# atenpas/gpd

Hardware: AMD Instinct MI355X
Metric: 15-ch grasp candidates scored/sec (imagegen+LeNet) at 1/2/4/8 MI355X (higher is better)
Workload: dtype f64 geometry / u8 images / LeNet f32-equivalent by exact operand splitting: conv1 int8 digit planes of 32-bit fixed-point weights (i32 accumulate, exact), conv2 + ip1 three bf16 pieces per operand (six exact products per term, f32 accumulate), ip2 f32

## Files before the change

### gpd_amd/api.py

```python
import ctypes as C
import os
import subprocess

import numpy as np

_HERE = os.path.dirname(os.path.abspath(__file__))
LIB_PATH = os.environ.get("GPD_HIP_LIB") or os.path.join(_HERE, "libgpd_hip.so")
_LIB = None

HAND_DTYPE = np.dtype([
    ("sample", "<f8", (3,)), ("frame", "<f8", (9,)), ("position", "<f8", (3,)),
    ("top", "<f8"), ("bottom", "<f8"), ("center", "<f8"), ("grasp_width", "<f8"),
    ("score", "<f4"), ("finger_placement_index", "<i4"), ("set_index", "<i4"), ("slot", "<i4"),
    ("valid", "u1"), ("half_antipodal", "u1"), ("full_antipodal", "u1"), ("pad_", "u1", (5,)),
], align=False)


class Params(C.Structure):
    _fields_ = [
        ("finger_width", C.c_double), ("hand_outer_diameter", C.c_double), ("hand_depth", C.c_double),
        ("hand_height", C.c_double), ("init_bite", C.c_double), ("volume_width", C.c_double),
        ("volume_depth", C.c_double), ("volume_height", C.c_double), ("nn_radius_frames", C.c_double),
        ("friction_coeff", C.c_double), ("min_aperture", C.c_double), ("max_aperture", C.c_double),
        ("workspace_grasps", C.c_double * 6), ("image_size", C.c_int32), ("image_num_channels", C.c_int32),
# ... 126 lines not shown
    rc = lib().gpd_hip_sis_select(_ptr(cen) if len(cen) else None, len(cen), _ptr(g) if len(g) else None, len(g),
                                  _ptr(u) if len(u) else None, len(u), _ptr(lst) if lst is not None and len(lst) else None,
                                  0 if lst is None else len(lst), _ptr(xyz) if len(xyz) else None, len(xyz), _ptr(ws),
                                  int(sampling_method), int(num_gauss), int(num_rand), _ptr(samples), _ptr(acc), _ptr(used), C.byref(short))
    if rc != 0:
        raise GpdHipError("libgpd_hip error %d: %s" % (rc, lib().gpd_hip_last_error().decode()))
    return dict(samples=samples[:n].copy(), accepted=acc, consumed=used, shortfall=int(short.value))


class ImageModel(C.Structure):
    _fields_ = [("window_class", C.c_int32), ("set_sd", C.c_int32), ("set_sr", C.c_int32), ("num_shadow", C.c_int32),
                ("stride_a", C.c_uint32), ("stride_c", C.c_uint32), ("true_div", C.c_int32), ("reserved_", C.c_int32),
                ("thr", (C.c_double * 61) * 3)]


def image_model(params):
    m = ImageModel()
    rc = lib().gpd_hip_image_model(C.byref(params), C.byref(m))
    if rc != 0:
        raise GpdHipError("libgpd_hip error %d: %s" % (rc, lib().gpd_hip_last_error().decode()))
    out = {k: int(getattr(m, k)) for k in ("window_class", "set_sd", "set_sr", "num_shadow", "stride_a", "stride_c", "true_div")}
    out["thr"] = np.array(m.thr, np.float64).reshape(3, 61)
    return out


TORCH_KEYS = ("conv1.weight", "conv1.bias", "conv2.weight", "conv2.bias", "fc1.weight", "fc1.bias", "fc2.weight", "fc2.bias")


def torch_state_arrays(state):
    plain = {}
    for k, v in state.items():
        k = str(k)
        plain[k[len("module."):] if k.startswith("module.") else k] = v
    out = {}
    for k in TORCH_KEYS:
        if k not in plain:
            raise KeyError("state dict has no %r (keys: %s)" % (k, sorted(plain)))
        v = plain[k]
        if hasattr(v, "detach"):
            v = v.detach().cpu().numpy()
        out[k] = np.ascontiguousarray(v, np.float32)
    return out


def lenet_from_torch(state, channels, input_scale=1.0 / 256):
    t = torch_state_arrays(state)
# ... 86 lines not shown
    if rc != 0:
        raise GpdHipError("libgpd_hip error %d: %s" % (rc, L.gpd_hip_last_error().decode()))
    return shape, outs


def bind_host_thread(device):
    n = C.c_int(0)
    node = lib().gpd_hip_bind_host_thread(int(device), C.byref(n))
    return int(node), int(n.value)


EXPORTS = ["gpd_hip_default_params", "gpd_hip_create", "gpd_hip_destroy", "gpd_hip_last_error",
           "gpd_hip_set_lenet_weights", "gpd_hip_score", "gpd_hip_upload_cloud", "gpd_hip_search",
           "gpd_hip_images", "gpd_hip_detect", "gpd_hip_last_stage_ms", "gpd_hip_replay", "gpd_hip_replay_times", "gpd_hip_last_images_stats", "gpd_hip_estimate_normals",
           "gpd_hip_search_samples", "gpd_hip_detect_samples", "gpd_hip_reevaluate", "gpd_hip_replay_kernel_ms", "gpd_hip_last_centre_chains",
           "gpd_hip_detect_select", "gpd_hip_detect_batch", "gpd_hip_detect_batch_multi", "gpd_hip_conv1_stats", "gpd_hip_last_fallbacks", "gpd_hip_preprocess_cloud", "gpd_hip_find_clusters", "gpd_hip_reserve", "gpd_hip_bind_host_thread",
           "gpd_hip_set_lenet_mode", "gpd_hip_lenet_debug", "gpd_hip_lenet_fast_tables", "gpd_hip_detect_sharded",
           "gpd_hip_sample_above_plane", "gpd_hip_last_image_routes", "gpd_hip_refine_normals", "gpd_hip_sample_positions",
           "gpd_hip_set_lenet_conv_relu", "gpd_hip_lenet_from_torch",
           "gpd_hip_lenet_shape_check", "gpd_hip_lenet_net_from_torch", "gpd_hip_set_lenet_net", "gpd_hip_lenet_net_debug",
           "gpd_hip_lenet_net_info", "gpd_hip_set_lenet_net_mode", "gpd_hip_bf16_split3",
           "gpd_hip_upload_ground_truth", "gpd_hip_label_view", "gpd_hip_balance_view", "gpd_hip_sizeof_label_view_job",
           "gpd_hip_shuffle_orders", "gpd_hip_sis_proposals", "gpd_hip_sis_select", "gpd_hip_detect_sis", "gpd_hip_sizeof_sis_job",
           "gpd_hip_image_model", "gpd_hip_given_check", "gpd_hip_images_given", "gpd_hip_score_given",
           "gpd_hip_train_default_params", "gpd_hip_train_create", "gpd_hip_train_destroy", "gpd_hip_train_init_state",
           "gpd_hip_train_set_state", "gpd_hip_train_get_state", "gpd_hip_train_set_data", "gpd_hip_train_steps",
           "gpd_hip_train_gradients", "gpd_hip_train_apply", "gpd_hip_train_eval", "gpd_hip_train_step_timed",
           "gpd_hip_train_kernel_name", "gpd_hip_sizeof_train_recipe", "gpd_hip_train_default_recipe", "gpd_hip_train_create_recipe",
           "gpd_hip_train_init_xavier", "gpd_hip_train_learning_rate", "gpd_hip_train_get_solver_state",
           "gpd_hip_train_set_solver_state", "gpd_hip_train_kernel_name_of",
           "gpd_hip_train_reserve", "gpd_hip_train_count", "gpd_hip_train_append_data", "gpd_hip_train_get_data",
           "gpd_hip_train_reorder", "gpd_hip_train_append_view",
           "gpd_hip_train_group_mean", "gpd_hip_train_group_slices", "gpd_hip_train_group_schedule", "gpd_hip_train_group_create",
           "gpd_hip_train_group_destroy", "gpd_hip_train_group_broadcast", "gpd_hip_train_group_steps", "gpd_hip_train_group_verify",
           "gpd_hip_train_group_last_bytes",
           "gpd_hip_train_create_net", "gpd_hip_train_shape", "gpd_hip_train_net_set_state", "gpd_hip_train_net_get_state",
           "gpd_hip_train_net_gradients", "gpd_hip_train_net_apply", "gpd_hip_train_net_get_solver_state",
           "gpd_hip_train_net_set_solver_state", "gpd_hip_train_net_sizes", "gpd_hip_train_net_init_state",
           "gpd_hip_train_net_init_xavier"]


def build(prof=True):
    subprocess.check_call(["make", "-s", "-j4", "-C", os.path.join(_HERE, "csrc")])
    if prof:
        subprocess.check_call(["make", "-s", "-j4", "-C", os.path.join(_HERE, "csrc"), "prof"])


# ... 43 lines not shown
        L.gpd_hip_reserve.argtypes = [C.c_void_p, C.c_int, C.c_int, C.c_int, C.c_int, C.c_int]
        L.gpd_hip_bind_host_thread.argtypes = [C.c_int, C.POINTER(C.c_int)]
        L.gpd_hip_set_lenet_mode.argtypes = [C.c_void_p, C.c_int]
        L.gpd_hip_set_lenet_conv_relu.argtypes = [C.c_void_p, C.c_int]
        L.gpd_hip_lenet_from_torch.argtypes = [C.c_int, C.c_double] + [C.c_void_p] * 6
        L.gpd_hip_lenet_debug.argtypes = [C.c_void_p, C.c_int, C.c_int, C.c_void_p]
        L.gpd_hip_lenet_shape_check.argtypes = [C.POINTER(LenetShape)]
        L.gpd_hip_lenet_net_from_torch.argtypes = [C.POINTER(LenetShape), C.c_double, C.c_void_p, C.c_void_p]
        L.gpd_hip_set_lenet_net.argtypes = [C.c_void_p, C.POINTER(LenetShape), C.c_void_p]
        L.gpd_hip_lenet_net_debug.argtypes = [C.c_void_p, C.c_int, C.c_int, C.c_void_p]
        L.gpd_hip_lenet_net_info.argtypes = [C.c_void_p, C.c_void_p]
        L.gpd_hip_set_lenet_net_mode.argtypes = [C.c_void_p, C.c_int]
        L.gpd_hip_bf16_split3.argtypes = [C.c_void_p, C.c_longlong, C.c_void_p, C.c_void_p, C.c_void_p]
        L.gpd_hip_replay_times.argtypes = [C.c_void_p, C.c_void_p, C.POINTER(C.c_int), C.c_void_p]
        L.gpd_hip_upload_ground_truth.argtypes = [C.c_void_p, C.c_void_p, C.c_void_p, C.c_int]
        L.gpd_hip_label_view.argtypes = [C.c_void_p, C.POINTER(LabelViewJob)]
        L.gpd_hip_balance_view.argtypes = [C.c_void_p, C.c_int, C.c_int, C.c_void_p, C.POINTER(C.c_int), C.POINTER(C.c_int)]
        L.gpd_hip_shuffle_orders.argtypes = [C.c_uint32, C.c_void_p, C.c_int, C.c_void_p]
        L.gpd_hip_sis_proposals.argtypes = [C.c_uint32, C.c_int, C.c_int, C.c_longlong, C.c_int, C.c_double, C.c_void_p]
        L.gpd_hip_sis_select.argtypes = [C.c_void_p, C.c_int, C.c_void_p, C.c_int, C.c_void_p, C.c_int, C.c_void_p, C.c_int, C.c_void_p, C.c_int,
                                         C.c_void_p, C.c_int, C.c_int, C.c_int, C.c_void_p, C.c_void_p, C.c_void_p, C.POINTER(C.c_int)]
        L.gpd_hip_detect_sis.argtypes = [C.c_void_p, C.POINTER(SisJob)]
        L.gpd_hip_image_model.argtypes = [C.POINTER(Params), C.POINTER(ImageModel)]
        L.gpd_hip_given_check.argtypes = [C.POINTER(Params), C.c_void_p, C.c_int, C.POINTER(C.c_int), C.POINTER(C.c_int)]
        L.gpd_hip_images_given.argtypes = [C.c_void_p, C.c_void_p, C.c_int, C.c_uint64, C.c_void_p, C.c_void_p, C.POINTER(C.c_int),
                                           C.POINTER(C.c_uint64)]
        L.gpd_hip_score_given.argtypes = [C.c_void_p, C.c_void_p, C.c_int, C.c_uint64, C.c_void_p, C.c_void_p, C.POINTER(C.c_int),
                                          C.POINTER(C.c_uint64)]
        L.gpd_hip_train_default_params.argtypes = [C.POINTER(TrainParams)]
        L.gpd_hip_train_default_params.restype = None
        L.gpd_hip_train_create.argtypes = [C.c_void_p, C.POINTER(TrainParams), C.POINTER(C.c_void_p)]
        L.gpd_hip_train_destroy.argtypes = [C.c_void_p]
        L.gpd_hip_train_destroy.restype = None
        L.gpd_hip_train_init_state.argtypes = [C.c_int, C.c_uint32, C.POINTER(C.c_void_p)]
        L.gpd_hip_train_set_state.argtypes = [C.c_void_p, C.POINTER(C.c_void_p)]
        L.gpd_hip_train_get_state.argtypes = [C.c_void_p, C.POINTER(C.c_void_p)]
        L.gpd_hip_train_set_data.argtypes = [C.c_void_p, C.c_int, C.c_void_p, C.c_void_p, C.c_int]
        L.gpd_hip_train_steps.argtypes = [C.c_void_p, C.c_void_p, C.c_int, C.c_int, C.c_void_p]
        L.gpd_hip_train_gradients.argtypes = [C.c_void_p, C.c_void_p, C.c_int, C.POINTER(C.c_void_p), C.POINTER(C.c_float)]
        L.gpd_hip_train_apply.argtypes = [C.c_void_p, C.POINTER(C.c_void_p)]
        L.gpd_hip_train_eval.argtypes = [C.c_void_p, C.c_int, C.c_void_p, C.c_int, C.c_void_p, C.POINTER(C.c_int)]
        L.gpd_hip_train_step_timed.argtypes = [C.c_void_p, C.c_void_p, C.c_int, C.c_void_p, C.c_int, C.POINTER(C.c_int)]
        L.gpd_hip_train_kernel_name.argtypes = [C.c_int]
        L.gpd_hip_train_kernel_name.restype = C.c_char_p
        L.gpd_hip_train_default_recipe.argtypes = [C.POINTER(TrainRecipe), C.c_int]
        L.gpd_hip_train_create_recipe.argtypes = [C.c_void_p, C.POINTER(TrainParams), C.POINTER(TrainRecipe), C.POINTER(C.c_void_p)]
# ... 874 lines not shown
```

### gpd_amd/csrc/image_device.h

```cpp
#pragma once
#include <cfloat>
#include <type_traits>

#include "gpd_internal.h"
#include "image_model.h"
#include "wave_ops.h"

namespace gpd {

static_assert(kImgCells == kImg, "image_model.h and gpd_internal.h disagree about the image size");
constexpr int IMG_THREADS = 512;
constexpr int IMG_WAVES = IMG_THREADS / 64;

struct Box {
  double F[9];
  double sample[3];
  double off[3];
  double lo[3], hi[3];
};

struct PointArrays {
  double t[3][PT_CAP];
  float4 an[PT_CAP];
};
// ... 73 lines not shown
  const int h = pr == 2 ? cx : cy;
  return h + v * kImg;
}
__device__ inline int depth_axis(int pr) { return pr == 0 ? 2 : (pr == 1 ? 0 : 1); }

__device__ inline double div_len(double x, int axis) {
  const ImgConsts &K = c_img;
  if (K.true_div) return x / K.len[axis];
  const double y = K.inv_len[axis];
  const double q = x * y;
  const double r = __builtin_fma(-K.len[axis], q, x);
  return __builtin_fma(r, y, q);
}
template <int NTAB>
__device__ inline double recip_count(const double *tab, float fc) {
  const int k = (int)fc;
  return k < NTAB ? tab[k] : 1.0 / (double)fc;
}

__device__ inline uint32_t lcg_step(uint32_t &s) {
  s = 214013u * s + 2531011u;
  return (uint32_t)(((int32_t)s >> 16) & 0x7FFF);
}
__device__ inline uint32_t lcg_jump(uint32_t s, unsigned long long n) {
  const image::LcgMap m = image::lcg_affine(n);
  return m.a * s + m.c;
}

template <class SM>
__device__ inline int block_excl_scan(SM &S, int v, int *total) {
  const int lane = threadIdx.x & 63, wave = threadIdx.x >> 6;
  const int incl = wave_incl_scan_i32(v);
  if (lane == 63) S.red_i[wave] = incl;
  __syncthreads();
  int base = 0, tot = 0;
#pragma unroll
  for (int w = 0; w < IMG_WAVES; w++) {
    const int x = S.red_i[w];
    if (w < wave) base += x;
    tot += x;
  }
  *total = tot;
  return base + incl - v;
}

template <class SM>
__device__ int scan_cells(SM &S) {
  const int tid = threadIdx.x;
  constexpr int PER = 8;
  static_assert(kPix % PER == 0 && kPix / PER <= IMG_THREADS, "scan_cells: cells per thread");
// ... 404 lines not shown
```

### gpd_amd/csrc/image_model.h

```cpp
#pragma once
#include <cfloat>
#include <cmath>
#include <cstddef>
#include <cstdint>
#include <cstdio>
#include <cstring>
#include <mutex>

#include "../../include/gpd_hip.h"

namespace gpd {

constexpr int kImgCells = 60;

constexpr int SET_THREADS = 1024;
constexpr int PT_CAP = 1024;
constexpr int PT_CAP_BIG = 32768;
constexpr int SH_CAP = 6144;
constexpr int SH_CAP_BIG = 12288;
template <bool WIDE>
struct Vox {
  static constexpr int VD = WIDE ? 64 : 46;
  static constexpr int SD = WIDE ? 128 : 86;
  static constexpr int SR = WIDE ? 64 : 43;
  static constexpr int LB = 18;
  static constexpr int SETWORDS = (SD * SD * SD + 31) / 32;
};
constexpr int LGRID = 256;
constexpr size_t PTS_SCRATCH_BYTES = (size_t)PT_CAP_BIG * (3 * sizeof(double) + 4 * sizeof(float) + sizeof(uint32_t));
constexpr int HUGE_CAP = 65535;
constexpr int HUGE_WIN = 256;
constexpr size_t HUGE_SCRATCH_BYTES = (size_t)HUGE_WIN * HUGE_WIN * sizeof(int32_t) + (size_t)(HUGE_CAP + 1) * (2 * sizeof(uint32_t) + sizeof(uint16_t)) + 64;

struct ImgConsts {
  double vol_depth, vol_width, vol_height, half_od, dbl_h;
  int C, nproj, per;
  double shadow_length, voxel, voxel_mult, rand_inv;
  int num_shadow;
  uint32_t stride_a, stride_c;
  double len[3];
  double inv_cell[3];
  double thr[3][kImgCells + 1];
  double inv_len[3];
  int true_div;
  int set_sd, set_sr;
};

namespace image {

struct LcgMap {
  uint32_t a, c;
};
constexpr LcgMap lcg_affine(unsigned long long n) {
  uint32_t a = 214013u, c = 2531011u, A = 1u, Cc = 0u;
  while (n) {
    if (n & 1ull) {
      A = a * A;
      Cc = a * Cc + c;
    }
    c = (a + 1u) * c;
    a = a * a;
    n >>= 1;
  }
  return LcgMap{A, Cc};
}

struct Window {
  bool wide = false;
  bool huge = false;
  int set_sd = 0, set_sr = 0;
  int cls() const { return huge ? 2 : (wide ? 1 : 0); }
};
inline int window_class(const gpd_params &p, Window &w, char *msg, size_t msg_len) {
  const double vox = 0.003;
  const double diag = std::sqrt(p.volume_depth * p.volume_depth + p.volume_width * p.volume_width + 4.0 * p.volume_height * p.volume_height);
  const double rx = std::fmax(p.hand_depth - p.init_bite, p.volume_depth);
  const double ry = 0.5 * (p.hand_outer_diameter - p.finger_width) + 0.5 * p.volume_width;
  const double reach = std::sqrt(rx * rx + ry * ry + p.volume_height * p.volume_height);
  const double need_win = std::ceil(diag / vox) + 3.0, need_reach = std::ceil(reach / vox) + 1.0;
  w.wide = need_win > (double)Vox<false>::VD || need_reach > (double)(Vox<false>::SR - 1);
  w.huge = need_win > (double)Vox<true>::VD || need_reach > (double)(Vox<true>::SR - 1);
  if (w.huge) {
    if (need_reach + 2.0 > 640.0) {
      snprintf(msg, msg_len, "images: an image volume with %.2f m of reach is beyond the shadow region this library allocates", reach);
      return GPD_ERR_CAPACITY;
    }
    w.set_sr = (int)need_reach + 2;
    w.set_sd = 2 * w.set_sr;
// ... 70 lines not shown
  k.num_shadow = (int)std::floor(k.shadow_length / k.voxel);
  k.len[0] = k.vol_depth;
  k.len[1] = k.vol_width;
  k.len[2] = k.dbl_h;
  k.true_div = 0;
  k.set_sd = w.set_sd;
  k.set_sr = w.set_sr;
  {
    static Axis cache[3];
    static std::mutex cache_mutex;
    std::lock_guard<std::mutex> lock(cache_mutex);
    for (int a = 0; a < 3; a++) {
      Axis &ac = cache[a];
      if (ac.len != k.len[a]) axis_model(k.len[a], ac);
      k.inv_cell[a] = (double)kImgCells / k.len[a];
      std::memcpy(k.thr[a], ac.thr, sizeof(ac.thr));
      k.inv_len[a] = ac.inv_len;
      if (ac.true_div) k.true_div = 1;
    }
  }
  const LcgMap stride = lcg_affine((unsigned long long)SET_THREADS * (unsigned)k.num_shadow);
  k.stride_a = stride.a;
  k.stride_c = stride.c;
}

}
}
```

### gpd_amd/csrc/image_state.hip

```cpp
#include <cstdio>
#include <cstring>

#include <vector>

#include "gpd_internal.h"
#include "buffers.h"
#include "image_model.h"

namespace gpd {

void images_free(ImageState &im) {
  device_release(im.d_images, im.d_images_hwc, im.d_status, im.d_set_bits, im.d_overflow, im.d_overflow2, im.d_pts_overflow, im.d_pts_scratch, im.d_huge_scratch);
  if (im.ev_fork) (void)hipEventDestroy(im.ev_fork);
  if (im.ev_join) (void)hipEventDestroy(im.ev_join);
  if (im.aux) (void)hipStreamDestroy(im.aux);
  im = ImageState();
}

int images_reserve(const gpd_params &p, ImageState &im, int n, int shadow_sets) {
  const int C = p.image_num_channels;
  if (!im.d_status) {
    HIP_RET(device_alloc(im.d_status, 4));
    HIP_RET(hipMemset(im.d_status, 0, 4 * sizeof(int32_t)));
    HIP_RET(device_alloc(im.d_pts_scratch, (size_t)LGRID * PTS_SCRATCH_BYTES));
// ... 126 lines not shown
    return GPD_ERR_INVALID;
  }
  image::Window w;
  char msg[160];
  const int rc = image::window_class(*params, w, msg, sizeof(msg));
  if (rc) {
    set_error("%s", msg);
    return rc;
  }
  ImgConsts k;
  image::fill_consts(*params, w, k);
  static_assert(sizeof(out->thr) == sizeof(k.thr), "gpd_image_model");
  out->window_class = w.cls();
  out->set_sd = k.set_sd;
  out->set_sr = k.set_sr;
  out->num_shadow = k.num_shadow;
  out->stride_a = k.stride_a;
  out->stride_c = k.stride_c;
  out->true_div = k.true_div;
  out->reserved_ = 0;
  std::memcpy(out->thr, k.thr, sizeof(k.thr));
  return GPD_OK;
}
```

### gpd_amd/csrc/images.hip

```cpp
#include <cfloat>
#include <cmath>
#include <cstddef>
#include <cstdio>
#include <cstdlib>
#include <cstring>

#include <mutex>

#include "const_block.h"
#include "gpd_internal.h"
#include "image_model.h"

namespace gpd {

__constant__ ImgConsts c_img;

struct ImgParams {
  const float *nn;
  int cap;
  const double *centers;
  const gpd_hand *hands;
  const int32_t *cand_hand;
  const int32_t *meta;
  const uint32_t *set_bits;
// ... 922 lines not shown
      __syncthreads();
      const int q = it / np;
      grasp_image_body<true>(P, S, P.cand_list[q], it - q * np);
    }
  } else {
    const int cand = xcd_candidate(P.num_cand);
    if (cand < 0) return;
    grasp_image_body<false>(P, S, cand);
  }
}

struct SetParams {
  const float *nn;
  int cap;
  const double *centers;
  const double *frames;
  const int32_t *set_meta;
  uint32_t *set_bits;
  const gpd_hand *hands;
  const int32_t *hand_cand;
  int slots;
  unsigned long long lcg_base;
  double view_point[3 * kMaxCams];
};

template <int MODE>
__global__ __launch_bounds__(SET_THREADS, MODE == 0 ? 8 : 1) void shadow_set_kernel(SetParams P) {
  constexpr bool WIDE = MODE != 0;
  const ImgConsts &K = c_img;
  const int SD = MODE == 2 ? K.set_sd : Vox<MODE == 1>::SD, SR = MODE == 2 ? K.set_sr : Vox<MODE == 1>::SR;
  const int SETWORDS = MODE == 2 ? (int)(((long long)SD * SD * SD + 31) / 32) : Vox<MODE == 1>::SETWORDS;
  __shared__ uint32_t lds_bits[WIDE ? 1 : Vox<false>::SETWORDS];
  __shared__ int s_bb[6];
  const int set = blockIdx.x;
  const int tid = threadIdx.x;
  const int slot_s = P.set_meta[8 * set + 0];
  const int N = P.set_meta[8 * set + 1];
  const unsigned long long off =
      P.lcg_base + (((unsigned long long)(uint32_t)P.set_meta[8 * set + 3] << 32) | (uint32_t)P.set_meta[8 * set + 2]);
  const int cam = P.set_meta[8 * set + 4];
  const float *nn = P.nn + (size_t)slot_s * 6 * P.cap;
  uint32_t *out = P.set_bits + (size_t)set * SETWORDS;
  uint32_t *bits = WIDE ? out : lds_bits;
  if (!WIDE) {
    if (tid == 0) {
      s_bb[0] = s_bb[2] = s_bb[4] = SD;
      s_bb[1] = s_bb[3] = s_bb[5] = -1;
    }
    for (int w = tid; w < SETWORDS; w += SET_THREADS) lds_bits[w] = 0u;
    __syncthreads();
  }
  const double *smp = P.frames + 12 * (size_t)slot_s;
  const int org[3] = {(int)floor(smp[0] * K.voxel_mult) - SR, (int)floor(smp[1] * K.voxel_mult) - SR,
                      (int)floor(smp[2] * K.voxel_mult) - SR};
  if (!WIDE) {
    if (tid < P.slots && P.hand_cand[(size_t)slot_s * P.slots + tid] >= 0) {
      const gpd_hand &H = P.hands[(size_t)slot_s * P.slots + tid];
      const double lo[3] = {H.bottom, H.center - K.half_od, -1.0 * K.vol_height};
      const double hi[3] = {H.bottom + K.vol_depth, H.center + K.half_od, K.vol_height};
      double wmin[3] = {DBL_MAX, DBL_MAX, DBL_MAX}, wmax[3] = {-DBL_MAX, -DBL_MAX, -DBL_MAX};
      for (int k = 0; k < 8; k++) {
        const double bx = (k & 1) ? hi[0] : lo[0], by = (k & 2) ? hi[1] : lo[1], bz = (k & 4) ? hi[2] : lo[2];
        for (int a = 0; a < 3; a++) {
          const double w = H.sample[a] + H.frame[3 * a] * bx + H.frame[3 * a + 1] * by + H.frame[3 * a + 2] * bz;
          wmin[a] = fmin(wmin[a], w);
          wmax[a] = fmax(wmax[a], w);
        }
      }
      for (int a = 0; a < 3; a++) {
        atomicMin(&s_bb[2 * a], (int)floor(wmin[a] * K.voxel_mult) - 1 - org[a]);
        atomicMax(&s_bb[2 * a + 1], (int)floor(wmax[a] * K.voxel_mult) + 1 - org[a]);
      }
    }
    __syncthreads();
  }
  const double *cen = P.centers + 3 * (size_t)slot_s;
  double vec[3];
  for (int r = 0; r < 3; r++) vec[r] = cen[r] - P.view_point[3 * cam + r];
  const double nrm = sqrt(vec[0] * vec[0] + vec[1] * vec[1] + vec[2] * vec[2]);
  for (int r = 0; r < 3; r++) vec[r] = K.shadow_length * vec[r] / nrm;
  uint32_t state = lcg_jump(0u, off + (unsigned long long)tid * (unsigned)K.num_shadow);
  int ox = org[0], oy = org[1], oz = org[2];
  asm volatile("" : "+v"(ox), "+v"(oy), "+v"(oz));
  auto draw_ray = [&](const double p0, const double p1, const double p2, uint32_t st) {
    for (int k = 0; k < K.num_shadow; k++) {
      const double t = (double)(int)lcg_step(st) * K.rand_inv;
      const int vx = (int)((p0 + t * vec[0]) * K.voxel_mult) - ox;
      const int vy = (int)((p1 + t * vec[1]) * K.voxel_mult) - oy;
      const int vz = (int)((p2 + t * vec[2]) * K.voxel_mult) - oz;
      if ((unsigned)vx < (unsigned)SD && (unsigned)vy < (unsigned)SD && (unsigned)vz < (unsigned)SD) {
        unsigned bit;
        asm("v_mad_u32_u24 %0, %1, %2, %3" : "=v"(bit) : "v"(vx), "s"(SD), "v"(vy));
        asm("v_mad_u32_u24 %0, %1, %2, %3" : "=v"(bit) : "v"(bit), "s"(SD), "v"(vz));
        atomicOr(&bits[bit >> 5], 1u << (bit & 31));
      }
    }
  };
  if constexpr (MODE == 0) {
    double wlo[3], whi[3], dinv[3];
    bool par[3];
#pragma unroll
    for (int a = 0; a < 3; a++) {
      const int b0 = max(s_bb[2 * a], 0), b1 = min(s_bb[2 * a + 1], SD - 1);
      wlo[a] = (double)(b0 + org[a] - 2);
// ... 21 lines not shown
          const double ta = (wlo[a] - q) * dinv[a], tb = (whi[a] - q) * dinv[a];
          t0 = fmax(t0, fmin(ta, tb));
          t1 = fmin(t1, fmax(ta, tb));
        }
      }
      keep = keep && t0 <= t1;
      const unsigned long long ballot = __ballot(keep);
      const int k = __popcll(ballot);
      if (k) {
        const int below = __popcll(ballot & ((1ull << lane) - 1ull));
        const int dest = ((keep ? pend + below : pend + k + (lane - below)) & 63) << 2;
        auto move = [dest](const double x) {
          return __hiloint2double(__builtin_amdgcn_ds_permute(dest, __double2hiint(x)),
                                  __builtin_amdgcn_ds_permute(dest, __double2loint(x)));
        };
        const double a0 = move(p0), a1 = move(p1), a2 = move(p2);
        const uint32_t as = (uint32_t)__builtin_amdgcn_ds_permute(dest, (int)state);
        const bool arrived = ((lane - pend) & 63) < k;
        if (pend + k < 64) {
          if (arrived) g0 = a0, g1 = a1, g2 = a2, gs = as;
          pend += k;
        } else {
          if (lane >= pend) g0 = a0, g1 = a1, g2 = a2, gs = as;
          draw_ray(g0, g1, g2, gs);
          pend += k - 64;
          if (lane < pend) g0 = a0, g1 = a1, g2 = a2, gs = as;
        }
      }
      state = K.stride_a * state + K.stride_c;
    }
    if (lane < pend) draw_ray(g0, g1, g2, gs);
  } else {
    for (int i = tid; i < N; i += SET_THREADS) {
      draw_ray((double)nn[0 * P.cap + i], (double)nn[1 * P.cap + i], (double)nn[2 * P.cap + i], state);
      state = K.stride_a * state + K.stride_c;
    }
  }
  if (!WIDE) {
    __syncthreads();
    const int x0 = max(s_bb[0], 0), x1 = min(s_bb[1], SD - 1), y0 = max(s_bb[2], 0), y1 = min(s_bb[3], SD - 1);
    if (x1 >= x0 && y1 >= y0) {
      const int wpr = (((y1 - y0 + 1) * SD + 31) >> 5) + 1;
      for (int idx = tid; idx < (x1 - x0 + 1) * wpr; idx += SET_THREADS) {
        const int x = x0 + idx / wpr, k = idx - (idx / wpr) * wpr;
        const int first = (x * SD + y0) * SD, last = (x * SD + y1 + 1) * SD - 1;
        const int w = (first >> 5) + k;
        if (w <= (last >> 5)) out[w] = lds_bits[w];
      }
    }
  }
}

__global__ void planar_to_hwc_kernel(const uint8_t *__restrict__ src, uint8_t *__restrict__ dst, int C, size_t total) {
  const size_t i = (size_t)blockIdx.x * blockDim.x + threadIdx.x;
  if (i >= total) return;
  const size_t per = (size_t)kPix * C;
  const size_t img = i / per, r = i - img * per;
  const int pix = (int)(r / C), c = (int)(r - (size_t)pix * C);
  dst[i] = src[img * per + (size_t)c * kPix + pix];
}
__global__ void hwc_to_planar_kernel(const uint8_t *__restrict__ src, uint8_t *__restrict__ dst, int C, size_t total) {
  const size_t i = (size_t)blockIdx.x * blockDim.x + threadIdx.x;
  if (i >= total) return;
  const size_t per = (size_t)kPix * C;
  const size_t img = i / per, r = i - img * per;
  const int c = (int)(r / kPix), pix = (int)(r - (size_t)c * kPix);
  dst[i] = src[img * per + (size_t)pix * C + c];
}
hipError_t planar_to_hwc(const uint8_t *src, uint8_t *dst, int n, int C, hipStream_t stream) {
  const size_t total = (size_t)n * kPix * C;
  if (!total) return hipSuccess;
  planar_to_hwc_kernel<<<(unsigned)((total + 255) / 256), 256, 0, stream>>>(src, dst, C, total);
// ... 68 lines not shown
    HIP_RET(hipGetLastError());
  }
  {
    ImgParams ip = base;
    ip.cand_list = pts_queue;
    ip.cand_count = pts_queued;
    ip.pts_scratch = im.d_pts_scratch;
    grasp_image_kernel<true><<<LGRID, IMG_THREADS, 0, pts_stream>>>(ip);
    HIP_RET(hipGetLastError());
  }
  if (im.num_shadow_sets > 0) {
    SetParams sp;
    sp.nn = s.d_nn;
    sp.cap = s.nn_cap;
    sp.centers = s.d_centers;
    sp.frames = s.d_frames;
    sp.set_meta = pl.d_set_meta;
    sp.set_bits = im.d_set_bits;
    sp.hands = s.d_hands;
    sp.hand_cand = pl.d_hand_cand;
    sp.slots = im.slots;
    sp.lcg_base = im.lcg_base;
    std::memcpy(sp.view_point, im.view_points, sizeof(sp.view_point));
    if (im.huge) {
      const size_t setwords = (size_t)(((long long)im.set_sd * im.set_sd * im.set_sd + 31) / 32);
      HIP_RET(hipMemsetAsync(im.d_set_bits, 0, (size_t)im.num_shadow_sets * setwords * sizeof(uint32_t), stream));
      shadow_set_kernel<2><<<im.num_shadow_sets, SET_THREADS, 0, stream>>>(sp);
    } else if (im.wide) {
      HIP_RET(hipMemsetAsync(im.d_set_bits, 0, (size_t)im.num_shadow_sets * Vox<true>::SETWORDS * sizeof(uint32_t), stream));
      shadow_set_kernel<1><<<im.num_shadow_sets, SET_THREADS, 0, stream>>>(sp);
    } else {
      shadow_set_kernel<0><<<im.num_shadow_sets, SET_THREADS, 0, stream>>>(sp);
    }
    HIP_RET(hipGetLastError());
  }
  if (im.channels == 15 && im.huge) {
    ImgParams ip = base;
    ip.huge_scratch = im.d_huge_scratch;
    shadow_image_any_kernel<<<LGRID, IMG_THREADS, 0, stream>>>(ip);
    HIP_RET(hipGetLastError());
  } else if (im.channels == 15 && im.wide) {
    {
      ImgParams ip = base;
      ip.overflow_list = sh_queue;
      ip.overflow_count = sh_queued;
      shadow_image_kernel<SH_CAP, true><<<all, IMG_THREADS, 0, stream>>>(ip);
// ... 26 lines not shown
    }
    {
      ImgParams ip = base;
      ip.cand_list = sh_queue;
      ip.cand_count = sh_queued;
      shadow_image_kernel<SH_CAP_BIG, false><<<LGRID, IMG_THREADS, 0, stream>>>(ip);
      HIP_RET(hipGetLastError());
    }
  }
  HIP_RET(hipEventRecord(im.ev_join, pts_stream));
  if (pts_stream != stream) HIP_RET(hipStreamWaitEvent(stream, im.ev_join, 0));
  if (dbg) {
    unsigned long long h[32];
    HIP_RET(hipMemcpyAsync(h, d_dbg, sizeof(h), hipMemcpyDeviceToHost, stream));
    HIP_RET(hipStreamSynchronize(stream));
    static const char *names[14] = {"sh_extract",  "sh_list",       "sh_sort_list",  "sh_max_read", "sh_final",
                                    "pts_collect", "pts_sort_list", "pts_walk_tail", "pts_final",   "sh_nnz_read",
                                    "sh_walk_loop", "pts_nnz_read", "pts_setup",     "pts_walk_loop"};
    unsigned long long tot = 0;
    for (int i = 0; i < 14; i++) tot += h[i];
    for (int i = 0; i < 14; i++)
      fprintf(stderr, "[img-timing] %-16s %10.1f kcycles/cand  %5.1f%%\n", names[i], (double)h[i] / n / 1e3,
              100.0 * h[i] / (double)tot);
    fprintf(stderr, "[img-timing] shadow voxels in box: max %llu mean %.0f; in-box points: max %llu mean %.0f\n", h[28],
            (double)h[29] / n, h[30], (double)h[31] / n);
  }
  return GPD_OK;
}

}
```

### gpd_amd/csrc/wave_ops.h

```cpp
#pragma once
#include <hip/hip_runtime.h>

namespace gpd {

template <int CTRL, int RMASK>
__device__ inline unsigned dpp_u32(unsigned x) {
  return (unsigned)__builtin_amdgcn_update_dpp((int)x, (int)x, CTRL, RMASK, 0xf, false);
}
template <int CTRL, int RMASK>
__device__ inline double dpp_f64(double x) {
  const unsigned long long b = (unsigned long long)__double_as_longlong(x);
  const unsigned lo = dpp_u32<CTRL, RMASK>((unsigned)b), hi = dpp_u32<CTRL, RMASK>((unsigned)(b >> 32));
  return __longlong_as_double((long long)(((unsigned long long)hi << 32) | lo));
}
template <int CTRL, int RMASK>
__device__ inline long long dpp_i64(long long x) {
  const unsigned long long b = (unsigned long long)x;
  const unsigned lo = dpp_u32<CTRL, RMASK>((unsigned)b), hi = dpp_u32<CTRL, RMASK>((unsigned)(b >> 32));
  return (long long)(((unsigned long long)hi << 32) | lo);
}
#define GPD_WAVE_REDUCE(v, OP, DPP)            \
  v = OP(v, (DPP<0xB1, 0xf>(v)));   \
  v = OP(v, (DPP<0x4E, 0xf>(v)));   \
  v = OP(v, (DPP<0x141, 0xf>(v)));      \
// ... 25 lines not shown


__device__ inline double uniform_f64(double v) {
  const unsigned long long b = (unsigned long long)__double_as_longlong(v);
  const unsigned lo = __builtin_amdgcn_readfirstlane((unsigned)b);
  const unsigned hi = __builtin_amdgcn_readfirstlane((unsigned)(b >> 32));
  return __longlong_as_double((long long)(((unsigned long long)hi << 32) | lo));
}

template <int CTRL, int RMASK>
__device__ inline float dpp_f32(float x) {
  return __uint_as_float(dpp_u32<CTRL, RMASK>(__float_as_uint(x)));
}
__device__ inline float lane63_f32(float v) { return __uint_as_float(lane63_u32(__float_as_uint(v))); }
__device__ inline float wave_max_f32(float v) {
  GPD_WAVE_REDUCE(v, fmaxf, dpp_f32);
  return lane63_f32(v);
}
__device__ inline float wave_min_f32(float v) {
  GPD_WAVE_REDUCE(v, fminf, dpp_f32);
  return lane63_f32(v);
}

__device__ inline int wave_incl_scan_i32(int v) {
  v += __builtin_amdgcn_update_dpp(0, v, 0x111, 0xf, 0xf, false);
  v += __builtin_amdgcn_update_dpp(0, v, 0x112, 0xf, 0xf, false);
  v += __builtin_amdgcn_update_dpp(0, v, 0x114, 0xf, 0xf, false);
  v += __builtin_amdgcn_update_dpp(0, v, 0x118, 0xf, 0xf, false);
  v += __builtin_amdgcn_update_dpp(0, v, 0x142, 0xa, 0xf, false);
  v += __builtin_amdgcn_update_dpp(0, v, 0x143, 0xc, 0xf, false);
  return v;
}

__device__ inline unsigned block_or(unsigned v, unsigned *s_tmp) {
  GPD_WAVE_REDUCE(v, op_or, dpp_u32);
  v = lane63_u32(v);
  __syncthreads();
  if ((threadIdx.x & 63) == 0) s_tmp[threadIdx.x >> 6] = v;
  __syncthreads();
  return s_tmp[0] | s_tmp[1] | s_tmp[2] | s_tmp[3];
}
__device__ inline double block_min(double v, double *s_tmp) {
  GPD_WAVE_REDUCE(v, op_min, dpp_f64);
  v = lane63_f64(v);
  __syncthreads();
  if ((threadIdx.x & 63) == 0) s_tmp[threadIdx.x >> 6] = v;
// ... 39 lines not shown
```

### include/gpd_hip.h

```cpp
#ifndef GPD_HIP_H_
#define GPD_HIP_H_

#include <stddef.h>
#include <stdint.h>

#ifdef __cplusplus
extern "C" {
#endif

#define GPD_MAX_SLOTS 24

#define GPD_OK 0
#define GPD_ERR_INVALID (-1)
#define GPD_ERR_HIP (-2)
#define GPD_ERR_CAPACITY (-3)
#define GPD_ERR_STATE (-4)

#define GPD_LENET_SPLIT 0
#define GPD_LENET_F32_CHAIN 1

typedef struct gpd_params {
  double finger_width;
  double hand_outer_diameter;
  double hand_depth;
// ... 120 lines not shown
  int32_t max_grasps_per_view;
  uint8_t *images;
  uint8_t *labels;
  gpd_hand *hands;
  int32_t *src_index;
  int32_t capacity;
  uint8_t *all_labels; int32_t all_labels_capacity;
  int32_t *round_counts;
  int32_t rounds_run, num_candidates, num_positives, num_out, num_positives_out;
  int32_t gt_neighbourhoods;
  int64_t d2h_bytes;
  float stage_ms[4];
} gpd_label_view_job;
int gpd_hip_label_view(gpd_hip_ctx *ctx, gpd_label_view_job *job);
int gpd_hip_sizeof_label_view_job(void);

typedef struct gpd_image_model {
  int32_t window_class, set_sd, set_sr, num_shadow;
  uint32_t stride_a, stride_c;
  int32_t true_div, reserved_;
  double thr[3][61];
} gpd_image_model;
int gpd_hip_image_model(const gpd_params *params, gpd_image_model *out);

typedef struct gpd_sis_proposal {
  uint64_t idx_raw;
  double off[3];
} gpd_sis_proposal;
int gpd_hip_sis_proposals(uint32_t seed, int round, int kind, long long first, int count, double sigma, void *out);

int gpd_hip_sis_select(const double *centres, int num_centres, const gpd_sis_proposal *gauss, int num_gauss_proposals,
                       const uint64_t *uniform, int num_uniform_proposals, const int32_t *uniform_list, int num_uniform_list,
                       const float *cloud_xyz, int num_points, const double *workspace, int sampling_method, int num_gauss, int num_rand,
                       double *samples, int32_t *accepted, int32_t *consumed, int *shortfall);

typedef struct gpd_sis_job {
  const int32_t *sample_indices;
  int32_t num_init_samples;
  int32_t num_iterations;
  int32_t num_samples;
  int32_t sampling_method;
  double prob_rand_samples;
  double sigma;
  double min_score;
  double workspace[6];
  int32_t min_inliers, remove_inliers;
// ... 187 lines not shown
```

Measured before the change: 2.320 million.

## Streamline shadow_set_kernel prologue with LCG jump tables and wave-reduced bounds

Each thread's per-thread LCG jump, previously an O(log n) affine power computation, is replaced by composing precomputed hi/lo jump tables held in constant memory with a single shared offset state. Hand bounding boxes are now computed by one wave with per-axis work items and wave min/max reductions instead of shared-memory atomics. The LDS clear uses 16-byte stores and is moved after the bounds step, and the copy-out loop is restructured per x row per wave. The change also adds profiling ticks and a host-side model that checks the table jump against the direct jump. The constant block grows by the two tables.

```diff
diff --git a/gpd_amd/api.py b/gpd_amd/api.py
--- a/gpd_amd/api.py
+++ b/gpd_amd/api.py
@@ -172,6 +172,14 @@
     out = {k: int(getattr(m, k)) for k in ("window_class", "set_sd", "set_sr", "num_shadow", "stride_a", "stride_c", "true_div")}
     out["thr"] = np.array(m.thr, np.float64).reshape(3, 61)
     return out
+
+
+def lcg_jump_model(num_shadow, off):
+    table, direct = np.empty(1024, np.uint32), np.empty(1024, np.uint32)
+    rc = lib().gpd_hip_lcg_jump_model(int(num_shadow), int(off) & (2 ** 64 - 1), _ptr(table), _ptr(direct))
+    if rc != 0:
+        raise GpdHipError("libgpd_hip error %d: %s" % (rc, lib().gpd_hip_last_error().decode()))
+    return table, direct
 
 
 TORCH_KEYS = ("conv1.weight", "conv1.bias", "conv2.weight", "conv2.bias", "fc1.weight", "fc1.bias", "fc2.weight", "fc2.bias")
@@ -304,7 +312,7 @@
            "gpd_hip_lenet_net_info", "gpd_hip_set_lenet_net_mode", "gpd_hip_bf16_split3",
            "gpd_hip_upload_ground_truth", "gpd_hip_label_view", "gpd_hip_balance_view", "gpd_hip_sizeof_label_view_job",
            "gpd_hip_shuffle_orders", "gpd_hip_sis_proposals", "gpd_hip_sis_select", "gpd_hip_detect_sis", "gpd_hip_sizeof_sis_job",
-           "gpd_hip_image_model", "gpd_hip_given_check", "gpd_hip_images_given", "gpd_hip_score_given",
+           "gpd_hip_image_model", "gpd_hip_lcg_jump_model", "gpd_hip_given_check", "gpd_hip_images_given", "gpd_hip_score_given",
            "gpd_hip_train_default_params", "gpd_hip_train_create", "gpd_hip_train_destroy", "gpd_hip_train_init_state",
            "gpd_hip_train_set_state", "gpd_hip_train_get_state", "gpd_hip_train_set_data", "gpd_hip_train_steps",
            "gpd_hip_train_gradients", "gpd_hip_train_apply", "gpd_hip_train_eval", "gpd_hip_train_step_timed",
@@ -394,6 +402,7 @@
                                          C.c_void_p, C.c_int, C.c_int, C.c_int, C.c_void_p, C.c_void_p, C.c_void_p, C.POINTER(C.c_int)]
         L.gpd_hip_detect_sis.argtypes = [C.c_void_p, C.POINTER(SisJob)]
         L.gpd_hip_image_model.argtypes = [C.POINTER(Params), C.POINTER(ImageModel)]
+        L.gpd_hip_lcg_jump_model.argtypes = [C.c_int32, C.c_uint64, C.c_void_p, C.c_void_p]
         L.gpd_hip_given_check.argtypes = [C.POINTER(Params), C.c_void_p, C.c_int, C.POINTER(C.c_int), C.POINTER(C.c_int)]
         L.gpd_hip_images_given.argtypes = [C.c_void_p, C.c_void_p, C.c_int, C.c_uint64, C.c_void_p, C.c_void_p, C.POINTER(C.c_int),
                                            C.POINTER(C.c_uint64)]
diff --git a/gpd_amd/csrc/image_device.h b/gpd_amd/csrc/image_device.h
--- a/gpd_amd/csrc/image_device.h
+++ b/gpd_amd/csrc/image_device.h
@@ -119,10 +119,6 @@
   s = 214013u * s + 2531011u;
   return (uint32_t)(((int32_t)s >> 16) & 0x7FFF);
 }
-__device__ inline uint32_t lcg_jump(uint32_t s, unsigned long long n) {
-  const image::LcgMap m = image::lcg_affine(n);
-  return m.a * s + m.c;
-}
 
 template <class SM>
 __device__ inline int block_excl_scan(SM &S, int v, int *total) {
diff --git a/gpd_amd/csrc/image_model.h b/gpd_amd/csrc/image_model.h
--- a/gpd_amd/csrc/image_model.h
+++ b/gpd_amd/csrc/image_model.h
@@ -32,20 +32,6 @@
 constexpr int HUGE_WIN = 256;
 constexpr size_t HUGE_SCRATCH_BYTES = (size_t)HUGE_WIN * HUGE_WIN * sizeof(int32_t) + (size_t)(HUGE_CAP + 1) * (2 * sizeof(uint32_t) + sizeof(uint16_t)) + 64;
 
-struct ImgConsts {
-  double vol_depth, vol_width, vol_height, half_od, dbl_h;
-  int C, nproj, per;
-  double shadow_length, voxel, voxel_mult, rand_inv;
-  int num_shadow;
-  uint32_t stride_a, stride_c;
-  double len[3];
-  double inv_cell[3];
-  double thr[3][kImgCells + 1];
-  double inv_len[3];
-  int true_div;
-  int set_sd, set_sr;
-};
-
 namespace image {
 
 struct LcgMap {
@@ -64,6 +50,37 @@
   }
   return LcgMap{A, Cc};
 }
+constexpr int kJumpTable = 32;
+static_assert(SET_THREADS == kJumpTable * kJumpTable, "jump_hi x jump_lo cover the threads of shadow_set_kernel");
+constexpr uint32_t lcg_compose_from_zero(uint32_t off_state, const LcgMap &hi, const LcgMap &lo) {
+  return lo.a * (hi.a * off_state + hi.c) + lo.c;
+}
+inline void lcg_jump_tables(int num_shadow, LcgMap *lo, LcgMap *hi) {
+  for (int i = 0; i < kJumpTable; i++) {
+    lo[i] = lcg_affine((unsigned long long)i * (unsigned)num_shadow);
+    hi[i] = lcg_affine((unsigned long long)kJumpTable * (unsigned long long)i * (unsigned)num_shadow);
+  }
+}
+
+}
+
+struct ImgConsts {
+  double vol_depth, vol_width, vol_height, half_od, dbl_h;
+  int C, nproj, per;
+  double shadow_length, voxel, voxel_mult, rand_inv;
+  int num_shadow;
+  uint32_t stride_a, stride_c;
+  image::LcgMap jump_lo[image::kJumpTable];
+  image::LcgMap jump_hi[image::kJumpTable];
+  double len[3];
+  double inv_cell[3];
+  double thr[3][kImgCells + 1];
+  double inv_len[3];
+  int true_div;
+  int set_sd, set_sr;
+};
+
+namespace image {
 
 struct Window {
   bool wide = false;
@@ -180,7 +197,8 @@
   const LcgMap stride = lcg_affine((unsigned long long)SET_THREADS * (unsigned)k.num_shadow);
   k.stride_a = stride.a;
   k.stride_c = stride.c;
-}
-
-}
-}
+  lcg_jump_tables(k.num_shadow, k.jump_lo, k.jump_hi);
+}
+
+}
+}
diff --git a/gpd_amd/csrc/image_state.hip b/gpd_amd/csrc/image_state.hip
--- a/gpd_amd/csrc/image_state.hip
+++ b/gpd_amd/csrc/image_state.hip
@@ -172,3 +172,19 @@
   std::memcpy(out->thr, k.thr, sizeof(k.thr));
   return GPD_OK;
 }
+
+extern "C" int gpd_hip_lcg_jump_model(int32_t num_shadow, uint64_t off, uint32_t *table_state, uint32_t *direct_state) {
+  using namespace gpd;
+  if (num_shadow < 0) {
+    set_error("gpd_hip_lcg_jump_model: bad argument");
+    return GPD_ERR_INVALID;
+  }
+  image::LcgMap lo[image::kJumpTable], hi[image::kJumpTable];
+  image::lcg_jump_tables(num_shadow, lo, hi);
+  const uint32_t off_state = image::lcg_affine(off).c;
+  for (int tid = 0; tid < SET_THREADS; tid++) {
+    if (table_state) table_state[tid] = image::lcg_compose_from_zero(off_state, hi[tid >> 5], lo[tid & 31]);
+    if (direct_state) direct_state[tid] = image::lcg_affine(off + (unsigned long long)tid * (unsigned)num_shadow).c;
+  }
+  return GPD_OK;
+}
diff --git a/gpd_amd/csrc/images.hip b/gpd_amd/csrc/images.hip
--- a/gpd_amd/csrc/images.hip
+++ b/gpd_amd/csrc/images.hip
@@ -968,7 +968,19 @@
   int slots;
   unsigned long long lcg_base;
   double view_point[3 * kMaxCams];
+  unsigned long long *dbg;
 };
+
+#ifdef GPD_PROFILING
+#define SET_TICK_INIT unsigned long long t_last = P.dbg ? __builtin_readcyclecounter() : 0
+#define SET_TICK(k) TICK(k)
+#else
+#define SET_TICK_INIT
+#define SET_TICK(k) \
+  do {              \
+  } while (0)
+#endif
+enum { SET_T_CLEAR = 14, SET_T_BOUNDS, SET_T_JUMP, SET_T_RAYS, SET_T_DRAWS, SET_T_COPY };
 
 template <int MODE>
 __global__ __launch_bounds__(SET_THREADS, MODE == 0 ? 8 : 1) void shadow_set_kernel(SetParams P) {
@@ -976,8 +988,9 @@
   const ImgConsts &K = c_img;
   const int SD = MODE == 2 ? K.set_sd : Vox<MODE == 1>::SD, SR = MODE == 2 ? K.set_sr : Vox<MODE == 1>::SR;
   const int SETWORDS = MODE == 2 ? (int)(((long long)SD * SD * SD + 31) / 32) : Vox<MODE == 1>::SETWORDS;
-  __shared__ uint32_t lds_bits[WIDE ? 1 : Vox<false>::SETWORDS];
+  __shared__ __attribute__((aligned(16))) uint32_t lds_bits[WIDE ? 1 : Vox<false>::SETWORDS];
   __shared__ int s_bb[6];
+  __shared__ uint32_t s_off_state;
   const int set = blockIdx.x;
   const int tid = threadIdx.x;
   const int slot_s = P.set_meta[8 * set + 0];
@@ -988,44 +1001,71 @@
   const float *nn = P.nn + (size_t)slot_s * 6 * P.cap;
   uint32_t *out = P.set_bits + (size_t)set * SETWORDS;
   uint32_t *bits = WIDE ? out : lds_bits;
-  if (!WIDE) {
-    if (tid == 0) {
-      s_bb[0] = s_bb[2] = s_bb[4] = SD;
-      s_bb[1] = s_bb[3] = s_bb[5] = -1;
-    }
-    for (int w = tid; w < SETWORDS; w += SET_THREADS) lds_bits[w] = 0u;
-    __syncthreads();
-  }
+  SET_TICK_INIT;
   const double *smp = P.frames + 12 * (size_t)slot_s;
   const int org[3] = {(int)floor(smp[0] * K.voxel_mult) - SR, (int)floor(smp[1] * K.voxel_mult) - SR,
                       (int)floor(smp[2] * K.voxel_mult) - SR};
   if (!WIDE) {
-    if (tid < P.slots && P.hand_cand[(size_t)slot_s * P.slots + tid] >= 0) {
-      const gpd_hand &H = P.hands[(size_t)slot_s * P.slots + tid];
-      const double lo[3] = {H.bottom, H.center - K.half_od, -1.0 * K.vol_height};
-      const double hi[3] = {H.bottom + K.vol_depth, H.center + K.half_od, K.vol_height};
-      double wmin[3] = {DBL_MAX, DBL_MAX, DBL_MAX}, wmax[3] = {-DBL_MAX, -DBL_MAX, -DBL_MAX};
-      for (int k = 0; k < 8; k++) {
-        const double bx = (k & 1) ? hi[0] : lo[0], by = (k & 2) ? hi[1] : lo[1], bz = (k & 4) ? hi[2] : lo[2];
-        for (int a = 0; a < 3; a++) {
-          const double w = H.sample[a] + H.frame[3 * a] * bx + H.frame[3 * a + 1] * by + H.frame[3 * a + 2] * bz;
-          wmin[a] = fmin(wmin[a], w);
-          wmax[a] = fmax(wmax[a], w);
+    if (tid < 64) {
+      int bmin[3] = {SD, SD, SD}, bmax[3] = {-1, -1, -1};
+      for (int item = tid; item < 3 * P.slots; item += 64) {
+        const int slot = item / 3, a = item - 3 * slot;
+        const bool live = P.hand_cand[(size_t)slot_s * P.slots + slot] >= 0;
+        const gpd_hand &H = P.hands[(size_t)slot_s * P.slots + slot];
+        const double lo[3] = {H.bottom, H.center - K.half_od, -1.0 * K.vol_height};
+        const double hi[3] = {H.bottom + K.vol_depth, H.center + K.half_od, K.vol_height};
+        const double hs = H.sample[a], f0 = H.frame[3 * a], f1 = H.frame[3 * a + 1], f2 = H.frame[3 * a + 2];
+        double wmin = DBL_MAX, wmax = -DBL_MAX;
+#pragma unroll
+        for (int k = 0; k < 8; k++) {
+          const double bx = (k & 1) ? hi[0] : lo[0], by = (k & 2) ? hi[1] : lo[1], bz = (k & 4) ? hi[2] : lo[2];
+          const double w = hs + f0 * bx + f1 * by + f2 * bz;
+          wmin = fmin(wmin, w);
+          wmax = fmax(wmax, w);
         }
-      }
-      for (int a = 0; a < 3; a++) {
-        atomicMin(&s_bb[2 * a], (int)floor(wmin[a] * K.voxel_mult) - 1 - org[a]);
-        atomicMax(&s_bb[2 * a + 1], (int)floor(wmax[a] * K.voxel_mult) + 1 - org[a]);
-      }
-    }
-    __syncthreads();
-  }
+        const int org_a = a == 0 ? org[0] : (a == 1 ? org[1] : org[2]);
+        const int v0 = (int)floor(wmin * K.voxel_mult) - 1 - org_a, v1 = (int)floor(wmax * K.voxel_mult) + 1 - org_a;
+#pragma unroll
+        for (int b = 0; b < 3; b++) {
+          if (live && b == a) {
+            bmin[b] = min(bmin[b], v0);
+            bmax[b] = max(bmax[b], v1);
+          }
+        }
+      }
+#pragma unroll
+      for (int b = 0; b < 3; b++) {
+        bmin[b] = wave_min_i32(bmin[b]);
+        bmax[b] = wave_max_i32(bmax[b]);
+      }
+      if (tid == 0) {
+#pragma unroll
+        for (int b = 0; b < 3; b++) {
+          s_bb[2 * b] = bmin[b];
+          s_bb[2 * b + 1] = bmax[b];
+        }
+      }
+    }
+    SET_TICK(SET_T_BOUNDS);
+    constexpr int W4 = Vox<false>::SETWORDS / 4;
+    uint4 *const lds4 = reinterpret_cast<uint4 *>(lds_bits);
+    for (int w = tid; w < W4; w += SET_THREADS) lds4[w] = make_uint4(0u, 0u, 0u, 0u);
+    if (tid < Vox<false>::SETWORDS - 4 * W4) lds_bits[4 * W4 + tid] = 0u;
+  }
+  SET_TICK(SET_T_CLEAR);
+  if ((tid >> 6) == 1) {
+    const image::LcgMap off_map = image::lcg_affine(((unsigned long long)__builtin_amdgcn_readfirstlane((uint32_t)(off >> 32)) << 32) |
+                                                    __builtin_amdgcn_readfirstlane((uint32_t)off));
+    if (tid == 64) s_off_state = off_map.c;
+  }
+  __syncthreads();
+  uint32_t state = image::lcg_compose_from_zero(s_off_state, K.jump_hi[tid >> 5], K.jump_lo[tid & 31]);
+  SET_TICK(SET_T_JUMP);
   const double *cen = P.centers + 3 * (size_t)slot_s;
   double vec[3];
   for (int r = 0; r < 3; r++) vec[r] = cen[r] - P.view_point[3 * cam + r];
   const double nrm = sqrt(vec[0] * vec[0] + vec[1] * vec[1] + vec[2] * vec[2]);
   for (int r = 0; r < 3; r++) vec[r] = K.shadow_length * vec[r] / nrm;
-  uint32_t state = lcg_jump(0u, off + (unsigned long long)tid * (unsigned)K.num_shadow);
   int ox = org[0], oy = org[1], oz = org[2];
   asm volatile("" : "+v"(ox), "+v"(oy), "+v"(oz));
   auto draw_ray = [&](const double p0, const double p1, const double p2, uint32_t st) {
@@ -1093,32 +1133,35 @@
           pend += k;
         } else {
           if (lane >= pend) g0 = a0, g1 = a1, g2 = a2, gs = as;
+          SET_TICK(SET_T_RAYS);
           draw_ray(g0, g1, g2, gs);
+          SET_TICK(SET_T_DRAWS);
           pend += k - 64;
           if (lane < pend) g0 = a0, g1 = a1, g2 = a2, gs = as;
         }
       }
       state = K.stride_a * state + K.stride_c;
     }
+    SET_TICK(SET_T_RAYS);
     if (lane < pend) draw_ray(g0, g1, g2, gs);
+    SET_TICK(SET_T_DRAWS);
   } else {
     for (int i = tid; i < N; i += SET_THREADS) {
       draw_ray((double)nn[0 * P.cap + i], (double)nn[1 * P.cap + i], (double)nn[2 * P.cap + i], state);
       state = K.stride_a * state + K.stride_c;
     }
+    SET_TICK(SET_T_DRAWS);
   }
   if (!WIDE) {
     __syncthreads();
     const int x0 = max(s_bb[0], 0), x1 = min(s_bb[1], SD - 1), y0 = max(s_bb[2], 0), y1 = min(s_bb[3], SD - 1);
     if (x1 >= x0 && y1 >= y0) {
-      const int wpr = (((y1 - y0 + 1) * SD + 31) >> 5) + 1;
-      for (int idx = tid; idx < (x1 - x0 + 1) * wpr; idx += SET_THREADS) {
-        const int x = x0 + idx / wpr, k = idx - (idx / wpr) * wpr;
+      for (int x = x0 + (tid >> 6); x <= x1; x += SET_THREADS / 64) {
         const int first = (x * SD + y0) * SD, last = (x * SD + y1 + 1) * SD - 1;
-        const int w = (first >> 5) + k;
-        if (w <= (last >> 5)) out[w] = lds_bits[w];
-      }
-    }
+        for (int w = (first >> 5) + (tid & 63); w <= (last >> 5); w += 64) out[w] = lds_bits[w];
+      }
+    }
+    SET_TICK(SET_T_COPY);
   }
 }
 
@@ -1233,6 +1276,7 @@
     sp.slots = im.slots;
     sp.lcg_base = im.lcg_base;
     std::memcpy(sp.view_point, im.view_points, sizeof(sp.view_point));
+    sp.dbg = dbg;
     if (im.huge) {
       const size_t setwords = (size_t)(((long long)im.set_sd * im.set_sd * im.set_sd + 31) / 32);
       HIP_RET(hipMemsetAsync(im.d_set_bits, 0, (size_t)im.num_shadow_sets * setwords * sizeof(uint32_t), stream));
@@ -1305,6 +1349,12 @@
     for (int i = 0; i < 14; i++)
       fprintf(stderr, "[img-timing] %-16s %10.1f kcycles/cand  %5.1f%%\n", names[i], (double)h[i] / n / 1e3,
               100.0 * h[i] / (double)tot);
+    static const char *set_names[6] = {"set_clear", "set_bounds", "set_jump", "set_rays", "set_draws", "set_copy"};
+    unsigned long long set_tot = 0;
+    for (int i = 0; i < 6; i++) set_tot += h[SET_T_CLEAR + i];
+    for (int i = 0; i < 6 && set_tot; i++)
+      fprintf(stderr, "[img-timing] %-16s %10.1f kcycles/set   %5.1f%%\n", set_names[i],
+              (double)h[SET_T_CLEAR + i] / (im.num_shadow_sets > 0 ? im.num_shadow_sets : 1) / 1e3, 100.0 * h[SET_T_CLEAR + i] / (double)set_tot);
     fprintf(stderr, "[img-timing] shadow voxels in box: max %llu mean %.0f; in-box points: max %llu mean %.0f\n", h[28],
             (double)h[29] / n, h[30], (double)h[31] / n);
   }
diff --git a/gpd_amd/csrc/wave_ops.h b/gpd_amd/csrc/wave_ops.h
--- a/gpd_amd/csrc/wave_ops.h
+++ b/gpd_amd/csrc/wave_ops.h
@@ -71,6 +71,19 @@
   return lane63_f32(v);
 }
 
+__device__ inline unsigned op_imin(unsigned a, unsigned b) { return (unsigned)min((int)a, (int)b); }
+__device__ inline unsigned op_imax(unsigned a, unsigned b) { return (unsigned)max((int)a, (int)b); }
+__device__ inline int wave_min_i32(int x) {
+  unsigned v = (unsigned)x;
+  GPD_WAVE_REDUCE(v, op_imin, dpp_u32);
+  return (int)lane63_u32(v);
+}
+__device__ inline int wave_max_i32(int x) {
+  unsigned v = (unsigned)x;
+  GPD_WAVE_REDUCE(v, op_imax, dpp_u32);
+  return (int)lane63_u32(v);
+}
+
 __device__ inline int wave_incl_scan_i32(int v) {
   v += __builtin_amdgcn_update_dpp(0, v, 0x111, 0xf, 0xf, false);
   v += __builtin_amdgcn_update_dpp(0, v, 0x112, 0xf, 0xf, false);
diff --git a/include/gpd_hip.h b/include/gpd_hip.h
--- a/include/gpd_hip.h
+++ b/include/gpd_hip.h
@@ -166,6 +166,7 @@
   double thr[3][61];
 } gpd_image_model;
 int gpd_hip_image_model(const gpd_params *params, gpd_image_model *out);
+int gpd_hip_lcg_jump_model(int32_t num_shadow, uint64_t off, uint32_t *table_state, uint32_t *direct_state);
 
 typedef struct gpd_sis_proposal {
   uint64_t idx_raw;
```

Result: no change. 2.327 million (median of 2 runs) (+0.3%).
